# thunlp/OpenMatch

Measured on NVIDIA H100. Metric: queries/sec top-1000 over 8.8M x 768 corpus, higher is better.
Workload: dtype f16

## Files before the change

### openmatch_b200/csrc/scan_gemm.cuh

```cuda
#pragma once
#include <cuda_fp16.h>

#include "scan_epilogue.cuh"

namespace om {

constexpr int kScanBlockN = 256;
constexpr int kScanStages = 3;
constexpr int kScanABytes = kBlockM * kBlockK * 2;
constexpr int kScanBBytes = kScanBlockN * kBlockK * 2;
constexpr int kScanStageBytes = kScanABytes + kScanBBytes;
constexpr int kScanConsumers = 256;
constexpr int kScanStash = 4;
constexpr int kScanStashOffset = kScanStages * kScanStageBytes;
constexpr int kScanStashBytes = 2 * 2 * kScanStash * kScanConsumers * 8;
constexpr int kScanBarOffset = kScanStashOffset + kScanStashBytes;
constexpr int kScanSmemBytes = kScanBarOffset + 2 * kScanStages * 8 + 1024;
static_assert(kScanSmemBytes <= 232448, "scan ring + stash exceed the 227 KB of shared memory an H100 block may use");

template <int H>
__device__ __forceinline__ float scan_pick(const float (&acc)[128], int i) {
  float a[32], b[16], c[8], d[4], e[2];
#pragma unroll
  for (int j = 0; j < 32; ++j) a[j] = (i & 1) ? acc[4 * j + 2 * H + 1] : acc[4 * j + 2 * H];
// ... 172 lines not shown
      const int row0 = m_blk * kBlockM + frow, row1 = row0 + 8;
      const float inf = __int_as_float(0x7f800000);
      const float t0 = row0 < nq ? thr[row0] : inf, t1 = row1 < nq ? thr[row1] : inf;

      float acc[128];
#pragma unroll
      for (int i = 0; i < 128; ++i) acc[i] = 0.f;
      ring_consume(
          full_bar, ring, 0, num_k, 31,
          [&](uint32_t stage, uint32_t accumulate) {
            const uint32_t a_addr = smem_u32(smem + stage * kScanStageBytes) + wg * (64 * 128);
            const uint32_t b_addr = smem_u32(smem + stage * kScanStageBytes + kScanABytes);
#pragma unroll
            for (int k = 0; k < kBlockK / kWgmmaK; ++k)
              wgmma_m64n256k16_f16<0, 0>(acc, wgmma_desc(a_addr + k * 32, kDescKMajorSW128),
                                         wgmma_desc(b_addr + k * 32, kDescKMajorSW128), (accumulate | k) != 0 ? 1u : 0u);
          },
          release);
      wgmma_fence_regs(acc);

      drain();
      const int col0 = n_blk * kScanBlockN;
      const int lim = n_cols - col0;
      unsigned long long* sb = stash + buf * (2 * kScanStash * kScanConsumers) + et;
      const int k0 = scan_filter_row<0>(acc, t0, row0, lim, q4, col0, sb, cand, count, overflow, C, row_base);
      const int k1 = scan_filter_row<1>(acc, t1, row1, lim, q4, col0, sb + kScanStash * kScanConsumers, cand, count,
                                        overflow, C, row_base);
      if (__any_sync(0xffffffffu, (k0 | k1) != 0)) {
        int x0 = k0, x1 = k1;
        int y0 = __shfl_up_sync(0xffffffffu, x0, 1, 4), y1 = __shfl_up_sync(0xffffffffu, x1, 1, 4);
        if (q4 >= 1) x0 += y0, x1 += y1;
        y0 = __shfl_up_sync(0xffffffffu, x0, 2, 4), y1 = __shfl_up_sync(0xffffffffu, x1, 2, 4);
        if (q4 >= 2) x0 += y0, x1 += y1;
        const int n0 = __shfl_sync(0xffffffffu, x0, lane | 3), n1 = __shfl_sync(0xffffffffu, x1, lane | 3);
        if (q4 == 0) {
          if (n0 > 0) p_pos0 = atomicAdd(count + row0, n0);
          if (n1 > 0) p_pos1 = atomicAdd(count + row1, n1);
        }
        p_n0 = k0;
        p_n1 = k1;
        p_excl0 = x0 - k0;
        p_excl1 = x1 - k1;
        p_row = row0;
        p_buf = buf;
        buf ^= 1;
      }
    }
    drain();
  }

  __syncthreads();
  cluster_sync_all();
}

template <int CQ, int CX>
static inline cudaError_t scan_wide_max_clusters(int num_sms, int* out) {
  static int max_clusters = -1;
  if (max_clusters < 0) {
    constexpr int kSize = ScanCluster<CQ, CX>::kSize;
    cudaError_t e =
        cudaFuncSetAttribute(scan_wide_kernel<CQ, CX>, cudaFuncAttributeMaxDynamicSharedMemorySize, kScanSmemBytes);
    if (e != cudaSuccess) return e;
    cudaLaunchConfig_t cfg = {};
    cfg.gridDim = dim3(kSize * (num_sms / kSize));
    cfg.blockDim = dim3(kGemmProducerThreads + kScanConsumers);
    cfg.dynamicSmemBytes = kScanSmemBytes;
    cudaLaunchAttribute attr[1];
    attr[0].id = cudaLaunchAttributeClusterDimension;
    attr[0].val.clusterDim = {static_cast<unsigned>(kSize), 1, 1};
    cfg.attrs = attr;
    cfg.numAttrs = 1;
    int n = 0;
    e = cudaOccupancyMaxActiveClusters(&n, scan_wide_kernel<CQ, CX>, &cfg);
    if (e != cudaSuccess) return e;
    max_clusters = n < num_sms / kSize ? n : num_sms / kSize;
  }
  *out = max_clusters;
  return cudaSuccess;
}

template <int CQ, int CX>
static inline cudaError_t launch_scan_wide(const __half* Q, int64_t ldq, const __half* X, int64_t ldx, int nq, int n_cols,
                                           int K, const float* thr, unsigned long long* cand, int* count, int* overflow,
                                           int C, uint32_t row_base, int num_sms, cudaStream_t stream) {
  using Cl = ScanCluster<CQ, CX>;
  CUtensorMap tmQ, tmX;
  if (make_tmap_bf16_2d(&tmQ, Q, (uint64_t)K, (uint64_t)nq, (uint64_t)ldq * 2, kBlockK, Cl::kQRows) != 0)
    return cudaErrorInvalidValue;
  if (make_tmap_bf16_2d(&tmX, X, (uint64_t)K, (uint64_t)n_cols, (uint64_t)ldx * 2, kBlockK, Cl::kXRows) != 0)
    return cudaErrorInvalidValue;
  int max_clusters = 0;
  cudaError_t e = scan_wide_max_clusters<CQ, CX>(num_sms, &max_clusters);
  if (e != cudaSuccess) return e;
  if (max_clusters < 1) return cudaErrorNotSupported;
  cudaLaunchConfig_t cfg = {};
  cfg.blockDim = dim3(kGemmProducerThreads + kScanConsumers);
  cfg.dynamicSmemBytes = kScanSmemBytes;
  cfg.stream = stream;
  cudaLaunchAttribute attr[1];
  attr[0].id = cudaLaunchAttributeClusterDimension;
  attr[0].val.clusterDim = {static_cast<unsigned>(Cl::kSize), 1, 1};
  cfg.attrs = attr;
  cfg.numAttrs = 1;
  const int qgroups = (nq + CQ * kBlockM - 1) / (CQ * kBlockM);
  const int64_t num_tiles = static_cast<int64_t>(qgroups) * ((n_cols + CX * kScanBlockN - 1) / (CX * kScanBlockN));
  const int clusters = num_tiles < max_clusters ? static_cast<int>(num_tiles) : max_clusters;
  cfg.gridDim = dim3(Cl::kSize * clusters);
  return cudaLaunchKernelEx(&cfg, scan_wide_kernel<CQ, CX>, tmQ, tmX, K, thr, cand, count, overflow, nq, n_cols, C,
                            row_base);
}

static inline cudaError_t launch_scan_cluster(int cq, int cx, const __half* Q, int64_t ldq, const __half* X, int64_t ldx,
                                              int nq, int n_cols, int K, const float* thr, unsigned long long* cand,
                                              int* count, int* overflow, int C, uint32_t row_base, int num_sms,
                                              cudaStream_t stream) {
  if (nq <= 0 || n_cols <= 0 || K <= 0) return cudaSuccess;
  if (cq == 2 && cx == 1)
    return launch_scan_wide<2, 1>(Q, ldq, X, ldx, nq, n_cols, K, thr, cand, count, overflow, C, row_base, num_sms, stream);
  if (cq == 4 && cx == 1)
    return launch_scan_wide<4, 1>(Q, ldq, X, ldx, nq, n_cols, K, thr, cand, count, overflow, C, row_base, num_sms, stream);
  if (cq == 2 && cx == 2)
    return launch_scan_wide<2, 2>(Q, ldq, X, ldx, nq, n_cols, K, thr, cand, count, overflow, C, row_base, num_sms, stream);
  if (cq == 4 && cx == 2)
    return launch_scan_wide<4, 2>(Q, ldq, X, ldx, nq, n_cols, K, thr, cand, count, overflow, C, row_base, num_sms, stream);
  return cudaErrorInvalidValue;
}

static inline cudaError_t scan_cluster_capacity(int cq, int cx, int num_sms, int* out) {
  *out = -1;
  if (cq == 2 && cx == 1) return scan_wide_max_clusters<2, 1>(num_sms, out);
  if (cq == 4 && cx == 1) return scan_wide_max_clusters<4, 1>(num_sms, out);
  if (cq == 2 && cx == 2) return scan_wide_max_clusters<2, 2>(num_sms, out);
  if (cq == 4 && cx == 2) return scan_wide_max_clusters<4, 2>(num_sms, out);
  return cudaSuccess;
}

}
```

### openmatch_b200/csrc/search.cu

```cuda
#include <cuda_fp16.h>
#include <float.h>
#include <math.h>
#include <stdlib.h>
#include <string.h>

#include <algorithm>
#include <new>
#include <vector>

#include "common.h"
#include "gemm.cuh"
#include "nccl_dyn.h"
#include "scan_epilogue.cuh"
#include "scan_gemm.cuh"

namespace om {

__device__ __forceinline__ void bitonic_sort_desc(unsigned long long* s, int P, int tid, int nthreads) {
  for (int k = 2; k <= P; k <<= 1) {
    for (int j = k >> 1; j > 0; j >>= 1) {
      for (int t = tid; t < (P >> 1); t += nthreads) {
        const int i = ((t & ~(j - 1)) << 1) | (t & (j - 1));
        const int p = i | j;
        const unsigned long long a = s[i], b = s[p];
// ... 460 lines not shown
                                   float* __restrict__ dst) {
  for (int64_t i = blockIdx.x * static_cast<int64_t>(blockDim.x) + threadIdx.x; i < static_cast<int64_t>(n) * d;
       i += static_cast<int64_t>(gridDim.x) * blockDim.x) {
    const int r = static_cast<int>(i / d);
    dst[i] = src[static_cast<size_t>(list[r]) * d + (i - static_cast<int64_t>(r) * d)];
  }
}
__global__ void scatter_results_kernel(const float* __restrict__ Dsub, const int64_t* __restrict__ Isub,
                                       const int* __restrict__ list, int n, int k, float* __restrict__ D,
                                       int64_t* __restrict__ I) {
  for (int64_t i = blockIdx.x * static_cast<int64_t>(blockDim.x) + threadIdx.x; i < static_cast<int64_t>(n) * k;
       i += static_cast<int64_t>(gridDim.x) * blockDim.x) {
    const int r = static_cast<int>(i / k);
    const size_t o = static_cast<size_t>(list[r]) * k + (i - static_cast<int64_t>(r) * k);
    D[o] = Dsub[i];
    I[o] = Isub[i];
  }
}
__global__ void compose_list_kernel(const int* __restrict__ outer, const int* __restrict__ inner, int n, int* out) {
  const int i = blockIdx.x * blockDim.x + threadIdx.x;
  if (i < n) out[i] = outer[inner[i]];
}

}

using namespace om;

struct om_comm {
  void* nccl = nullptr;
  int rank = 0, world = 1;
};

namespace {

constexpr int kQueryChunk = 16384;
constexpr int kMaxCandidates = 4096;

struct DevBuf {
  void* p = nullptr;
  size_t bytes = 0;
  int reserve(size_t need) {
    if (need <= bytes) return 0;
    if (p) cudaFree(p);
    p = nullptr;
    bytes = 0;
    OM_CUDA(dev_malloc(&p, need));
    bytes = need;
    return 0;
  }
  void release() {
    if (p) cudaFree(p);
    p = nullptr;
    bytes = 0;
  }
};

struct Level {
  int nq = 0, k = 0, kp = 0, kp_target = 0, C = 0, growth = 2, mode = 0, world = 1, kc = 0, nqc_max = 0;
  const float* qf = nullptr;
  __half* qh = nullptr;
  float *hn = nullptr, *en = nullptr;
  unsigned long long* cand = nullptr;
  int* count = nullptr;
  float* thr = nullptr;
  int* status = nullptr;
  uint8_t *send = nullptr, *recv = nullptr;
};

}

struct om_index {
  int d = 0, dpad = 0;
  int storage = OM_F32;
  int64_t n = 0, cap = 0;
  float* xf = nullptr;
  __half* xh = nullptr;
  float* gstats = nullptr;
  bool gstats_stale = false;
  int64_t st_nonfinite = 0;
  int64_t rescore_slack = -1;
  int force_safe = 0;
  int pair_scan = 1;
  int scan_cq = 0, scan_cx = 0;
  int growth = 0;
  int certify = 1;
  int exact_only = 0;
  int stage_scores = 0;
  int64_t st_rounds = 0, st_retries = 0, st_capacity = 0, st_launches = 0;
  int64_t st_flagged = 0, st_flagged_wide = 0, st_exact = 0;
  int64_t st_scan_cluster = 0, st_scan_clusters = 0;
  int profile = 0;
  double st_scan_us = 0, st_select_us = 0, st_final_us = 0, st_other_us = 0;
  std::vector<cudaEvent_t> ev;
  std::vector<int> ev_kind;
  size_t ev_used = 0;
  DevBuf ws, ows, sws;
  int* h_status = nullptr;
};

static int index_grow(om_index* ix, int64_t need) {
  if (need <= ix->cap) return 0;
  int64_t ncap = std::max<int64_t>(need, ix->cap + ix->cap / 2);
  ncap = round_up(std::max<int64_t>(ncap, 1024), 256);
  float* nxf = nullptr;
  __half* nxh = nullptr;
  const bool master = ix->storage == OM_F32;
  OM_CUDA(cudaDeviceSynchronize());
  if (master) OM_CUDA(dev_malloc(&nxf, static_cast<size_t>(ncap) * ix->d * sizeof(float)));
  cudaError_t e = dev_malloc(&nxh, static_cast<size_t>(ncap) * ix->dpad * sizeof(__half));
  if (e != cudaSuccess) {
    cudaFree(nxf);
    cudaGetLastError();
    return fail(OM_ENOMEM, "index: cannot allocate the fp16 rows for %lld rows", (long long)ncap);
  }
  if (ix->n > 0) {
    if (master)
      OM_CUDA(cudaMemcpy(nxf, ix->xf, static_cast<size_t>(ix->n) * ix->d * sizeof(float), cudaMemcpyDeviceToDevice));
    OM_CUDA(cudaMemcpy(nxh, ix->xh, static_cast<size_t>(ix->n) * ix->dpad * sizeof(__half), cudaMemcpyDeviceToDevice));
  }
  OM_CUDA(cudaDeviceSynchronize());
  cudaFree(ix->xf);
  cudaFree(ix->xh);
  ix->xf = nxf;
  ix->xh = nxh;
  ix->cap = ncap;
  return 0;
}

static inline int grid_for(int64_t n, int threads) {
  int64_t g = (n + threads - 1) / threads;
  return static_cast<int>(std::min<int64_t>(std::max<int64_t>(g, 1), 132 * 16));
}

static int settle_reset(om_index* ix, cudaStream_t st) {
  if (!ix->gstats_stale) return 0;
  OM_CUDA(cudaMemsetAsync(ix->gstats, 0, 3 * sizeof(float), st));
  ix->gstats_stale = false;
  return 0;
}

extern "C" {

int om_index_create(int d, om_index** out) { return om_index_create_typed(d, OM_F32, out); }

int om_index_create_typed(int d, om_dtype storage, om_index** out) {
  if (!out || d <= 0) return fail(OM_EINVAL, "om_index_create: d must be positive");
  if (storage != OM_F32 && storage != OM_F16)
    return fail(OM_EINVAL, "om_index_create_typed: storage must be OM_F32 or OM_F16 (the scan operand is fp16)");
  OM_TRY(device_sm_count());
  om_index* ix = new (std::nothrow) om_index();
  if (!ix) return fail(OM_ENOMEM, "om_index_create: out of host memory");
  ix->d = d;
  ix->dpad = static_cast<int>(round_up(d, 8));
  ix->storage = storage;
  if (cudaMalloc(&ix->gstats, 4 * sizeof(float)) != cudaSuccess || cudaMemset(ix->gstats, 0, 4 * sizeof(float)) != cudaSuccess ||
      cudaHostAlloc(&ix->h_status, 8 * sizeof(int), cudaHostAllocDefault) != cudaSuccess) {
    cudaGetLastError();
    cudaFree(ix->gstats);
    delete ix;
    return fail(OM_ENOMEM, "om_index_create: cannot allocate index state");
  }
  *out = ix;
  return 0;
}

void om_index_destroy(om_index* ix) {
  if (!ix) return;
  cudaFree(ix->xf);
  cudaFree(ix->xh);
  cudaFree(ix->gstats);
  if (ix->h_status) cudaFreeHost(ix->h_status);
  ix->ws.release();
  ix->ows.release();
  ix->sws.release();
  for (cudaEvent_t e : ix->ev) cudaEventDestroy(e);
  delete ix;
}

int64_t om_index_ntotal(const om_index* ix) { return ix ? ix->n : 0; }
int om_index_dim(const om_index* ix) { return ix ? ix->d : 0; }
int om_index_storage(const om_index* ix) { return ix ? ix->storage : fail(OM_EINVAL, "om_index_storage: null index"); }

int om_index_reset(om_index* ix) {
  if (!ix) return fail(OM_EINVAL, "om_index_reset: null index");
  ix->n = 0;
  ix->gstats_stale = true;
  ix->st_nonfinite = 0;
  return 0;
}

int om_index_reserve_rows(om_index* ix, int64_t n, void** dev_rows, int64_t* row_pitch_elems) {
  if (!ix || n < 0 || !dev_rows || !row_pitch_elems) return fail(OM_EINVAL, "om_index_reserve_rows: bad arguments");
  if (ix->n + n > 0xfffffff0ll) return fail(OM_EINVAL, "index shard limited to 2^32-16 rows; shard the corpus");
  OM_TRY(index_grow(ix, ix->n + n));
  if (ix->storage == OM_F16) {
    *dev_rows = ix->xh + static_cast<size_t>(ix->n) * ix->dpad;
    *row_pitch_elems = ix->dpad;
  } else {
    *dev_rows = ix->xf + static_cast<size_t>(ix->n) * ix->d;
    *row_pitch_elems = ix->d;
  }
  return 0;
}

int om_index_reserve(om_index* ix, int64_t n, float** dev_rows) {
  if (!ix || n < 0 || !dev_rows) return fail(OM_EINVAL, "om_index_reserve: bad arguments");
  if (ix->storage != OM_F32) return fail(OM_ESTATE, "om_index_reserve: the index stores fp16 rows; use om_index_reserve_rows");
  void* rows = nullptr;
  int64_t pitch = 0;
  OM_TRY(om_index_reserve_rows(ix, n, &rows, &pitch));
  *dev_rows = static_cast<float*>(rows);
  return 0;
}

int om_index_commit(om_index* ix, int64_t n, void* stream) {
  if (!ix || n < 0 || ix->n + n > ix->cap) return fail(OM_EINVAL, "om_index_commit: more rows than reserved");
  if (n == 0) return 0;
  cudaStream_t st = static_cast<cudaStream_t>(stream);
  OM_TRY(settle_reset(ix, st));
  if (ix->storage == OM_F16)
    commit_f16_rows_kernel<<<grid_for(n, 8), 256, 0, st>>>(ix->xh + static_cast<size_t>(ix->n) * ix->dpad, n, ix->d,
                                                           ix->dpad, ix->gstats, reinterpret_cast<int*>(ix->gstats) + 2);
  else
    rows_to_f16_kernel<<<grid_for(n, 8), 256, 0, st>>>(ix->xf + static_cast<size_t>(ix->n) * ix->d,
                                                       ix->xh + static_cast<size_t>(ix->n) * ix->dpad, n, ix->d, ix->dpad,
                                                       nullptr, nullptr, ix->gstats);
  OM_CUDA(cudaGetLastError());
  ix->n += n;
  return 0;
}

static int add_f16(om_index* ix, const void* x, om_memkind kind, om_dtype dtype, int64_t n, cudaStream_t st) {
  void* rows = nullptr;
  int64_t pitch = 0;
  OM_TRY(om_index_reserve_rows(ix, n, &rows, &pitch));
  __half* dst = static_cast<__half*>(rows);
  const size_t elems = static_cast<size_t>(n) * ix->d;
  const size_t esize = dtype == OM_F32 ? 4 : 2;
  const void* src = x;
  void* tmp = nullptr;
  if (kind == OM_HOST) {
    OM_CUDA(cudaMalloc(&tmp, elems * esize));
    OM_CUDA(cudaMemcpyAsync(tmp, x, elems * esize, cudaMemcpyHostToDevice, st));
    src = tmp;
  }
  int* bad = reinterpret_cast<int*>(ix->gstats) + 3;
  cudaError_t e = cudaMemsetAsync(bad, 0, sizeof(int), st);
  const int grid = grid_for(static_cast<int64_t>(elems), 256);
  if (e == cudaSuccess) {
    if (dtype == OM_F32)
      to_f16_rows_kernel<<<grid, 256, 0, st>>>(static_cast<const float*>(src), n, ix->d, dst, ix->dpad, bad);
    else if (dtype == OM_BF16)
      to_f16_rows_kernel<<<grid, 256, 0, st>>>(static_cast<const __nv_bfloat16*>(src), n, ix->d, dst, ix->dpad, bad);
    else
      to_f16_rows_kernel<<<grid, 256, 0, st>>>(static_cast<const __half*>(src), n, ix->d, dst, ix->dpad, bad);
    e = cudaGetLastError();
  }
  if (e == cudaSuccess) e = cudaMemcpyAsync(ix->h_status + 4, bad, sizeof(int), cudaMemcpyDeviceToHost, st);
  if (e == cudaSuccess) e = cudaStreamSynchronize(st);
  if (tmp) cudaFree(tmp);
  OM_CUDA(e);
  if (ix->h_status[4] > 0)
    return fail(OM_EINVAL, "om_index_add: %d elements are NaN or round to +-inf in fp16 (|x| >= 65520); fp16 storage cannot "
                "hold them and no row was added", ix->h_status[4]);
  return om_index_commit(ix, n, st);
}

int om_index_add(om_index* ix, const void* x, om_memkind kind, om_dtype dtype, int64_t n, void* stream) {
  if (!ix || (!x && n > 0) || n < 0) return fail(OM_EINVAL, "om_index_add: bad arguments");
  if (n == 0) return 0;
  cudaStream_t st = static_cast<cudaStream_t>(stream);
  if (ix->storage == OM_F16) {
    if (dtype != OM_F32 && dtype != OM_BF16 && dtype != OM_F16)
      return fail(OM_EINVAL, "om_index_add: unsupported dtype %d", (int)dtype);
    return add_f16(ix, x, kind, dtype, n, st);
  }
  float* dst = nullptr;
  OM_TRY(om_index_reserve(ix, n, &dst));
  const size_t elems = static_cast<size_t>(n) * ix->d;
  if (dtype == OM_F32) {
    OM_CUDA(cudaMemcpyAsync(dst, x, elems * 4, kind == OM_HOST ? cudaMemcpyHostToDevice : cudaMemcpyDeviceToDevice,
                            st));
  } else if (dtype == OM_BF16 || dtype == OM_F16) {
    const void* src = x;
    void* tmp = nullptr;
    if (kind == OM_HOST) {
      OM_CUDA(cudaMalloc(&tmp, elems * 2));
      OM_CUDA(cudaMemcpyAsync(tmp, x, elems * 2, cudaMemcpyHostToDevice, st));
      src = tmp;
    }
    if (dtype == OM_BF16)
      to_f32<<<grid_for(elems, 256), 256, 0, st>>>(static_cast<const __nv_bfloat16*>(src), dst, (int64_t)elems);
    else
      to_f32<<<grid_for(elems, 256), 256, 0, st>>>(static_cast<const __half*>(src), dst, (int64_t)elems);
    OM_CUDA(cudaGetLastError());
    if (tmp) {
      OM_CUDA(cudaStreamSynchronize(st));
      cudaFree(tmp);
    }
  } else {
    return fail(OM_EINVAL, "om_index_add: unsupported dtype %d", (int)dtype);
  }
  OM_TRY(om_index_commit(ix, n, stream));
  if (kind == OM_HOST) OM_CUDA(cudaStreamSynchronize(st));
  return 0;
}

int om_index_set_param(om_index* ix, const char* name, int64_t value) {
  if (!ix || !name) return fail(OM_EINVAL, "om_index_set_param: bad arguments");
  if (!strcmp(name, "rescore_slack")) {
    ix->rescore_slack = value;
  } else if (!strcmp(name, "force_safe_rounds")) {
    ix->force_safe = value != 0;
  } else if (!strcmp(name, "round_growth")) {
    if (value != 0 && (value < 2 || value > 8)) return fail(OM_EINVAL, "round_growth must be 0 (auto) or in [2, 8]");
    ix->growth = static_cast<int>(value);
  } else if (!strcmp(name, "pair_scan")) {
    ix->pair_scan = value != 0;
  } else if (!strcmp(name, "scan_cluster_q")) {
    if (value != 0 && value != 2 && value != 4) return fail(OM_EINVAL, "scan_cluster_q must be 0 (auto), 2 or 4");
    ix->scan_cq = static_cast<int>(value);
  } else if (!strcmp(name, "scan_cluster_x")) {
    if (value != 0 && value != 1 && value != 2) return fail(OM_EINVAL, "scan_cluster_x must be 0 (auto), 1 or 2");
    ix->scan_cx = static_cast<int>(value);
  } else if (!strcmp(name, "profile")) {
    ix->profile = static_cast<int>(value);
  } else if (!strcmp(name, "certify")) {
    ix->certify = value != 0;
  } else if (!strcmp(name, "exact_only")) {
    ix->exact_only = value != 0;
  } else if (!strcmp(name, "debug_stage_scores")) {
    ix->stage_scores = value != 0;
  } else {
    return fail(OM_EINVAL, "om_index_set_param: unknown parameter '%s'", name);
  }
  return 0;
}

int64_t om_index_get_stat(const om_index* ix, const char* name) {
  if (!ix || !name) return -1;
  if (!strcmp(name, "rounds")) return ix->st_rounds;
  if (!strcmp(name, "overflow_retries")) return ix->st_retries;
  if (!strcmp(name, "candidates")) return ix->st_capacity;
  if (!strcmp(name, "launches")) return ix->st_launches;
  if (!strcmp(name, "uncertified")) return ix->st_flagged;
  if (!strcmp(name, "uncertified_wide")) return ix->st_flagged_wide;
  if (!strcmp(name, "exact_queries")) return ix->st_exact;
  if (!strcmp(name, "nonfinite_rows")) return ix->st_nonfinite;
  if (!strcmp(name, "scan_cluster")) return ix->st_scan_cluster;
  if (!strcmp(name, "scan_max_clusters")) return ix->st_scan_clusters;
  if (!strcmp(name, "scan_ns")) return static_cast<int64_t>(ix->st_scan_us * 1e3);
  if (!strcmp(name, "select_ns")) return static_cast<int64_t>(ix->st_select_us * 1e3);
  if (!strcmp(name, "finalize_ns")) return static_cast<int64_t>(ix->st_final_us * 1e3);
  if (!strcmp(name, "other_ns")) return static_cast<int64_t>(ix->st_other_us * 1e3);
  return -1;
}

}

namespace {

struct Timed {
  om_index* ix;
  cudaStream_t st;
  bool on;
  Timed(om_index* ix_, cudaStream_t st_, int kind) : ix(ix_), st(st_), on(ix_->profile != 0) {
    static const char* nvtx_names[4] = {"om.search.scan", "om.search.select", "om.search.rescore", "om.search.exchange_certify"};
    nvtxRangePushA(nvtx_names[kind & 3]);
    if (!on) return;
    if (ix->ev_used + 2 > ix->ev.size()) {
      cudaEvent_t a, b;
      if (cudaEventCreate(&a) != cudaSuccess || cudaEventCreate(&b) != cudaSuccess) {
        on = false;
        return;
      }
      ix->ev.push_back(a);
      ix->ev.push_back(b);
      ix->ev_kind.push_back(0);
    }
    ix->ev_kind[ix->ev_used / 2] = kind;
    cudaEventRecord(ix->ev[ix->ev_used], st);
  }
  ~Timed() {
    nvtxRangePop();
    if (!on) return;
    cudaEventRecord(ix->ev[ix->ev_used + 1], st);
    ix->ev_used += 2;
  }
};

void collect_profile(om_index* ix) {
  static const char* names[4] = {"scan", "select", "finalize", "exchange+certify"};
  for (size_t i = 0; i + 1 < ix->ev_used; i += 2) {
    float ms = 0.f;
    if (cudaEventElapsedTime(&ms, ix->ev[i], ix->ev[i + 1]) != cudaSuccess) continue;
    const int kind = ix->ev_kind[i / 2];
    (kind == 0 ? ix->st_scan_us : kind == 1 ? ix->st_select_us : kind == 2 ? ix->st_final_us : ix->st_other_us) += ms * 1e3;
    if (ix->profile >= 2) fprintf(stderr, "[om profile] launch %zu %s %.3f ms\n", i / 2, names[kind & 3], ms);
  }
  ix->ev_used = 0;
}

int once_attrs() {
  static bool done = false;
  if (done) return 0;
  OM_CUDA(cudaFuncSetAttribute(select_kernel, cudaFuncAttributeMaxDynamicSharedMemorySize, 16384 * 8));
  OM_CUDA(cudaFuncSetAttribute(finalize_kernel<float>, cudaFuncAttributeMaxDynamicSharedMemorySize, kMaxCandidates * 8 + 65536));
  OM_CUDA(cudaFuncSetAttribute(finalize_kernel<__half>, cudaFuncAttributeMaxDynamicSharedMemorySize, kMaxCandidates * 8 + 65536));
  OM_CUDA(cudaFuncSetAttribute(merge_kernel, cudaFuncAttributeMaxDynamicSharedMemorySize, 8192 * 16));
  OM_CUDA(cudaFuncSetAttribute(exact_scan_kernel<8, 2, float>, cudaFuncAttributeMaxDynamicSharedMemorySize, 96 * 1024));
  OM_CUDA(cudaFuncSetAttribute(exact_scan_kernel<8, 2, __half>, cudaFuncAttributeMaxDynamicSharedMemorySize, 96 * 1024));
  done = true;
  return 0;
}

struct ExchangeBlock {
  size_t off_i, off_floor, off_stats, bytes;
};
inline ExchangeBlock exchange_block(size_t nqc, size_t kc) {
  ExchangeBlock b;
  b.off_i = round_up(nqc * kc * 4, 256);
  b.off_floor = b.off_i + round_up(nqc * kc * 8, 256);
  b.off_stats = b.off_floor + round_up(nqc * 4, 256);
  b.bytes = b.off_stats + 256;
  return b;
}
inline size_t exchange_block_bytes(size_t nqc, size_t kc) { return exchange_block(nqc, kc).bytes; }

int level_prepare(om_index* ix, Level& L, const float* qf, int nq, int k, int kp_target, int mode, int world,
                  cudaStream_t st) {
  const int d = ix->d, dpad = ix->dpad;
  if (d > 16384) return fail(OM_EINVAL, "om_index_search: d > 16384 unsupported");
  if (k > kMaxCandidates) return fail(OM_EINVAL, "om_index_search: k = %d exceeds %d", k, kMaxCandidates);
  OM_TRY(once_attrs());
  L.qf = qf;
  L.nq = nq;
  L.k = k;
  L.mode = mode;
  L.world = world;
  L.kp_target = std::min(std::max(kp_target, k), kMaxCandidates);
  if (world > 1 && mode == 0 && L.kp_target < kMaxCandidates) {
    const double m = static_cast<double>(L.kp_target) / world;
    L.kp_target = static_cast<int>(std::min<int64_t>(L.kp_target, round_up(static_cast<int64_t>(m + 6.0 * sqrt(m) + 32.0), 32)));
  }
  L.kp = static_cast<int>(std::min<int64_t>(L.kp_target, std::max<int64_t>(ix->n, 1)));
  for (L.growth = ix->growth > 0 ? ix->growth : (nq <= 256 ? 8 : 2);; --L.growth) {
    L.C = 1024;
    while (L.C < (5 * L.growth * L.kp) / 4 + 512) L.C <<= 1;
    if (L.C <= 16384 || L.growth == 2) break;
  }
  if (L.C > 16384) return fail(OM_EINVAL, "om_index_search: candidate list of %d entries exceeds 16384; lower k", L.C);
  L.kc = std::min(k, L.kp_target);
  L.nqc_max = std::min(nq, kQueryChunk);
  ix->st_capacity = L.C;
  size_t off = 0;
  auto carve = [&](size_t bytes) {
    size_t o = off;
    off += round_up(bytes, 256);
    return o;
  };
  const size_t nqc = L.nqc_max;
  const size_t o_qh = carve(static_cast<size_t>(nq) * dpad * 2), o_hn = carve(static_cast<size_t>(nq) * 4),
               o_en = carve(static_cast<size_t>(nq) * 4), o_cand = carve(nqc * L.C * 8), o_count = carve(nqc * 4),
               o_thr = carve(nqc * 4), o_status = carve(256);
  size_t o_send = 0, o_recv = 0;
  if (world > 1) {
    const size_t blk = exchange_block_bytes(nqc, L.kc);
    o_send = carve(blk);
    o_recv = carve(blk * world);
  }
  OM_TRY(ix->ws.reserve(off));
  uint8_t* base = static_cast<uint8_t*>(ix->ws.p);
  L.qh = reinterpret_cast<__half*>(base + o_qh);
  L.hn = reinterpret_cast<float*>(base + o_hn);
  L.en = reinterpret_cast<float*>(base + o_en);
  L.cand = reinterpret_cast<unsigned long long*>(base + o_cand);
  L.count = reinterpret_cast<int*>(base + o_count);
  L.thr = reinterpret_cast<float*>(base + o_thr);
  L.status = reinterpret_cast<int*>(base + o_status);
  L.send = world > 1 ? base + o_send : nullptr;
  L.recv = world > 1 ? base + o_recv : nullptr;
  if (mode == 0) {
    rows_to_f16_kernel<<<grid_for(nq, 8), 256, 0, st>>>(qf, L.qh, nq, d, dpad, L.hn, L.en, nullptr);
    OM_CUDA(cudaGetLastError());
    ix->st_launches += 1;
  }
  return 0;
}

int sweep_chunk(om_index* ix, const Level& L, int q0, int nqc, bool safe, int sms, cudaStream_t st) {
  const int64_t growth = L.growth;
  const int64_t N = ix->n;
  const int C = L.C, kp = L.kp;
  if (N == 0) {
    fill_i32<<<(nqc + 255) / 256, 256, 0, st>>>(L.count, 0, nqc);
    fill_i32<<<(nqc + 255) / 256, 256, 0, st>>>(reinterpret_cast<int*>(L.thr), static_cast<int>(0xff800000), nqc);
    OM_CUDA(cudaGetLastError());
    return 0;
  }
  const __half* qh = L.qh + static_cast<size_t>(q0) * ix->dpad;
  const float* qf = L.qf + static_cast<size_t>(q0) * ix->d;
  int* overflow = L.status;
  int64_t pos = 0;
  const size_t sel_smem = static_cast<size_t>(C) * 8;
  bool first = true;
  while (pos < N) {
    int64_t step;
    if (first)
      step = std::min<int64_t>(N, C);
    else if (safe)
      step = std::min<int64_t>(N - pos, std::max<int64_t>(256, ((C - kp) / 256) * 256));
    else
      step = std::min<int64_t>(N - pos, (growth - 1) * pos);
    {
      Timed t(ix, st, 0);
      if (L.mode == 0) {
        const __half* xrows = ix->xh + static_cast<size_t>(pos) * ix->dpad;
        cudaError_t e;
        const int ncols = static_cast<int>(step);
        const bool pair = ix->pair_scan != 0 && nqc > kBlockM;
        if (first) {
          EpiScan<true> epi{L.thr, L.cand, L.count, overflow, nqc, ncols, C, static_cast<uint32_t>(pos)};
          e = launch_gemm<128, 3, true, EpiScan<true>, true>(qh, ix->dpad, xrows, ix->dpad, nqc, ncols, ix->d, epi, sms, st, true);
        } else if (pair) {
          const int cq = ix->scan_cq ? ix->scan_cq : 2, cx = ix->scan_cx ? ix->scan_cx : 1;
          int clusters = 0;
          e = launch_scan_cluster(cq, cx, qh, ix->dpad, xrows, ix->dpad, nqc, ncols, ix->d, L.thr, L.cand, L.count,
                                  overflow, C, static_cast<uint32_t>(pos), sms, st);
          if (e == cudaSuccess) e = scan_cluster_capacity(cq, cx, sms, &clusters);
          ix->st_scan_cluster = 10 * cq + cx;
          ix->st_scan_clusters = clusters;
        } else {
          EpiScan<false> epi{L.thr, L.cand, L.count, overflow, nqc, ncols, C, static_cast<uint32_t>(pos)};
          e = launch_gemm<128, 3, true, EpiScan<false>, true>(qh, ix->dpad, xrows, ix->dpad, nqc, ncols, ix->d, epi, sms, st, true);
        }
        if (e != cudaSuccess) return fail(OM_ECUDA, "scan kernel launch failed: %s", cudaGetErrorString(e));
      } else {
        const int nqt = std::max(1, std::min(8, (96 * 1024) / (ix->d * 4)));
        dim3 grid(static_cast<unsigned>(std::min<int64_t>((step + 15) / 16, static_cast<int64_t>(sms) * 4)),
                  static_cast<unsigned>((nqc + nqt - 1) / nqt));
        const size_t smem = static_cast<size_t>(nqt) * ix->d * 4;
        if (ix->storage == OM_F16)
          exact_scan_kernel<8, 2><<<grid, 256, smem, st>>>(ix->xh + static_cast<size_t>(pos) * ix->dpad, step,
                                                           static_cast<uint32_t>(pos), qf, nqc, ix->d, nqt, L.thr, L.cand,
                                                           L.count, overflow, C, first ? 1 : 0);
        else
          exact_scan_kernel<8, 2><<<grid, 256, smem, st>>>(ix->xf + static_cast<size_t>(pos) * ix->d, step,
                                                           static_cast<uint32_t>(pos), qf, nqc, ix->d, nqt, L.thr, L.cand,
                                                           L.count, overflow, C, first ? 1 : 0);
        OM_CUDA(cudaGetLastError());
      }
    }
    {
      Timed t(ix, st, 1);
      select_kernel<<<nqc, 256, sel_smem, st>>>(L.cand, L.count, L.thr, C, kp, first ? static_cast<int>(step) : -1);
    }
    OM_CUDA(cudaGetLastError());
    ix->st_launches += 2;
    pos += step;
    first = false;
    ix->st_rounds++;
  }
  return 0;
}

int finalize_chunk(om_index* ix, const Level& L, int q0, int nqc, float* D, int64_t* I, int k_out, int64_t id_offset,
                   cudaStream_t st) {
  int P2 = 2;
  while (P2 < L.kp) P2 <<= 1;
  const size_t fin_smem = static_cast<size_t>(P2) * 8 + static_cast<size_t>(ix->d) * 4;
  {
    Timed t(ix, st, 2);
    const float* qf = L.qf + static_cast<size_t>(q0) * ix->d;
    if (ix->storage == OM_F16)
      finalize_kernel<<<nqc, 256, fin_smem, st>>>(L.cand, L.count, L.C, qf, ix->xh, ix->d, D, I, id_offset, k_out,
                                                  ix->stage_scores);
    else
      finalize_kernel<<<nqc, 256, fin_smem, st>>>(L.cand, L.count, L.C, qf, ix->xf, ix->d, D, I, id_offset, k_out,
                                                  ix->stage_scores);
  }
  OM_CUDA(cudaGetLastError());
  ix->st_launches += 1;
  return 0;
}

#define OM_NCCL(expr)                                                                                   \
  do {                                                                                                  \
    int r__ = (expr);                                                                                   \
    if (r__ != 0) return fail(OM_ECUDA, "%s failed: %s", #expr, nccl_api().GetErrorString(r__));        \
  } while (0)

int merge_parts(const float* Dp, const int64_t* Ip, int64_t stride_d, int64_t stride_i, int nparts, int nq, int k_in,
                int k_out, float* D, int64_t* I, cudaStream_t st) {
  OM_TRY(once_attrs());
  if (k_in > 8192) return fail(OM_EINVAL, "om_topk_merge_n: k_in = %d exceeds 8192", k_in);
  if (static_cast<int64_t>(nparts) * k_in <= 8192) {
    int P = 2;
    while (P < nparts * k_in) P <<= 1;
    const size_t smem = static_cast<size_t>(P) * 8 + static_cast<size_t>(nparts) * k_in * 8;
    merge_kernel<<<nq, 256, smem, st>>>(Dp, Ip, stride_d, stride_i, nparts, nq, k_in, k_out, D, I);
    OM_CUDA(cudaGetLastError());
    return 0;
  }
  if (k_in > 4096 || k_out > 4096)
    return fail(OM_EINVAL, "om_topk_merge_n: %d parts x %d entries exceed one merge of 8192 and need k_in, k_out <= 4096 "
                "(got k_in = %d, k_out = %d)", nparts, k_in, k_in, k_out);
  const int g = std::max(2, 8192 / k_in);
  const int ngroups = (nparts + g - 1) / g;
  const int k_mid = static_cast<int>(std::min<int64_t>(k_out, static_cast<int64_t>(g) * k_in));
  float* Dm = nullptr;
  int64_t* Im = nullptr;
  const size_t per = static_cast<size_t>(nq) * k_mid;
  OM_CUDA(cudaMallocAsync(&Dm, per * ngroups * 4, st));
  OM_CUDA(cudaMallocAsync(&Im, per * ngroups * 8, st));
// ... 27 lines not shown
  }
  ix->st_launches += 2;
  return 0;
}

int run_level(om_index* ix, om_comm* comm, Level& L, float* dD, int64_t* dI, int64_t id_offset, int* flags,
              int* flag_list, int* nflag_out, cudaStream_t st) {
  const int sms = device_sm_count();
  if (sms < 0) return sms;
  NvtxRange nvtx(L.mode == 1 ? "om.search.level_exact" : (L.kp_target >= kMaxCandidates ? "om.search.level_wide" : "om.search.level0"));
  const bool sharded = comm && comm->world > 1;
  bool safe = ix->force_safe != 0;
  const bool certify = ix->certify && L.mode == 0 && flags != nullptr && !ix->stage_scores;
  for (int attempt = 0; attempt < 4; ++attempt) {
    OM_CUDA(cudaMemsetAsync(L.status, 0, 32, st));
    for (int q0 = 0; q0 < L.nq; q0 += kQueryChunk) {
      const int nqc = std::min(kQueryChunk, L.nq - q0);
      OM_TRY(sweep_chunk(ix, L, q0, nqc, safe, sms, st));
      if (sharded)
        OM_TRY(exchange_chunk(ix, comm, L, q0, nqc, dD, dI, id_offset, st));
      else
        OM_TRY(finalize_chunk(ix, L, q0, nqc, dD + static_cast<size_t>(q0) * L.k, dI + static_cast<size_t>(q0) * L.k, L.k,
                              id_offset, st));
      if (certify) {
        Timed t(ix, st, 3);
        const ExchangeBlock b = exchange_block(nqc, L.kc);
        const float* floors = sharded ? reinterpret_cast<const float*>(L.recv + b.off_floor) : L.thr;
        const float* gst = sharded ? reinterpret_cast<const float*>(L.recv + b.off_stats) : ix->gstats;
        certify_kernel<<<(nqc + 7) / 8, 256, 0, st>>>(dD + static_cast<size_t>(q0) * L.k, dI + static_cast<size_t>(q0) * L.k,
                                                      L.k, floors, static_cast<int64_t>(b.bytes / 4), sharded ? comm->world : 1,
                                                      gst, static_cast<int64_t>(b.bytes / 4), L.hn + q0, L.en + q0, ix->d, nqc,
                                                      q0, flags, L.status + 2);
        OM_CUDA(cudaGetLastError());
        ix->st_launches += 1;
      }
    }
    if (sharded)
      OM_NCCL(nccl_api().AllReduce(L.status, L.status, 1, kNcclInt32, kNcclMax, comm->nccl, st));
    OM_CUDA(cudaMemcpyAsync(ix->h_status, L.status, 4 * sizeof(int), cudaMemcpyDeviceToHost, st));
    OM_CUDA(cudaStreamSynchronize(st));
    const unsigned int fault = read_clear_dev_fault();
    if (fault) return fail(OM_EFAULT, "scan kernel pipeline fault 0x%08x", fault);
    if (ix->h_status[0]) {
      if (safe) return fail(OM_EFAULT, "candidate list overflow in the overflow-proof schedule (bug)");
      safe = true;
      ix->st_retries++;
      continue;
    }
    *nflag_out = certify ? ix->h_status[2] : 0;
    if (*nflag_out > 0) {
      compact_flags_kernel<<<1, 1024, 0, st>>>(flags, L.nq, flag_list);
      OM_CUDA(cudaGetLastError());
      ix->st_launches += 1;
    }
    return 0;
  }
  return fail(OM_EFAULT, "search level did not converge (bug)");
}

int check_finite_rows(om_index* ix, om_comm* comm, cudaStream_t st) {
  if (ix->storage != OM_F16) return 0;
  int* cnt = reinterpret_cast<int*>(ix->gstats) + 2;
  const bool sharded = comm && comm->world > 1;
  if (sharded) OM_NCCL(nccl_api().AllReduce(cnt, cnt + 1, 1, kNcclInt32, kNcclSum, comm->nccl, st));
  OM_CUDA(cudaMemcpyAsync(ix->h_status + 4, cnt, 2 * sizeof(int), cudaMemcpyDeviceToHost, st));
  OM_CUDA(cudaStreamSynchronize(st));
  ix->st_nonfinite = ix->h_status[4];
  const int total = sharded ? ix->h_status[5] : ix->h_status[4];
  if (total > 0)
    return fail(OM_EINVAL, "search: %d committed fp16 rows hold inf or NaN (%d on this shard); fp16 storage cannot answer "
                "exactly over them: reset the index", total, ix->h_status[4]);
  return 0;
}

int search_impl(om_index* ix, om_comm* comm, const void* q, om_memkind q_kind, int nq, int k, float* D, int64_t* I,
                om_memkind out_kind, int64_t id_offset, cudaStream_t st) {
  NvtxRange nvtx("om.search");
  const int d = ix->d;
  const int world = comm ? comm->world : 1;
  ix->st_rounds = ix->st_retries = ix->st_launches = 0;
  ix->st_flagged = ix->st_flagged_wide = ix->st_exact = 0;
  ix->st_scan_cluster = ix->st_scan_clusters = 0;
  ix->st_scan_us = ix->st_select_us = ix->st_final_us = ix->st_other_us = 0;
  ix->ev_used = 0;
  OM_TRY(check_finite_rows(ix, comm, st));
  size_t off = 0;
  auto carve = [&](size_t bytes) {
    size_t o = off;
    off += round_up(bytes, 256);
    return o;
  };
  const size_t o_q = carve(q_kind == OM_HOST ? static_cast<size_t>(nq) * d * 4 : 0);
  const size_t o_D = carve(out_kind == OM_HOST ? static_cast<size_t>(nq) * k * 4 : 0);
  const size_t o_I = carve(out_kind == OM_HOST ? static_cast<size_t>(nq) * k * 8 : 0);
  const size_t o_flags = carve(static_cast<size_t>(nq) * 4);
  const size_t o_flag = carve(static_cast<size_t>(nq) * 4);
  const size_t o_sub = carve(static_cast<size_t>(nq) * 4);
  const size_t o_flag2 = carve(static_cast<size_t>(nq) * 4);
  OM_TRY(ix->ows.reserve(off));
  uint8_t* ob = static_cast<uint8_t*>(ix->ows.p);
  const float* qf = static_cast<const float*>(q);
  if (q_kind == OM_HOST) {
    OM_CUDA(cudaMemcpyAsync(ob + o_q, q, static_cast<size_t>(nq) * d * 4, cudaMemcpyHostToDevice, st));
    qf = reinterpret_cast<const float*>(ob + o_q);
  }
  float* dD = out_kind == OM_HOST ? reinterpret_cast<float*>(ob + o_D) : D;
  int64_t* dI = out_kind == OM_HOST ? reinterpret_cast<int64_t*>(ob + o_I) : I;
  int* flags = reinterpret_cast<int*>(ob + o_flags);
  int* flag_list = reinterpret_cast<int*>(ob + o_flag);
  int* sub_flags = reinterpret_cast<int*>(ob + o_sub);
  int* flag_list2 = reinterpret_cast<int*>(ob + o_flag2);

  const int64_t slack = ix->rescore_slack >= 0 ? ix->rescore_slack : std::max<int64_t>(128, k / 5);
  const int kp0 = static_cast<int>(std::min<int64_t>(static_cast<int64_t>(k) + slack, kMaxCandidates));
  int nf = 0;
  if (!ix->exact_only) {
    Level L;
    OM_TRY(level_prepare(ix, L, qf, nq, k, kp0, 0, world, st));
    OM_TRY(run_level(ix, comm, L, dD, dI, id_offset, flags, flag_list, &nf, st));
    ix->st_flagged = nf;
  }
  auto run_sub = [&](const int* list, int n_sub, int kp_target, int mode, int* nf_out) -> int {
    Level Ls;
    if (!list) {
      OM_TRY(level_prepare(ix, Ls, qf, n_sub, k, kp_target, mode, world, st));
      return run_level(ix, comm, Ls, dD, dI, id_offset, flags, sub_flags, nf_out, st);
    }
    size_t so = 0;
    auto scarve = [&](size_t bytes) {
      size_t o = so;
      so += round_up(bytes, 256);
      return o;
    };
    const size_t s_q = scarve(static_cast<size_t>(n_sub) * d * 4), s_D = scarve(static_cast<size_t>(n_sub) * k * 4),
                 s_I = scarve(static_cast<size_t>(n_sub) * k * 8);
    OM_TRY(ix->sws.reserve(so));
    uint8_t* sb = static_cast<uint8_t*>(ix->sws.p);
    float* qsub = reinterpret_cast<float*>(sb + s_q);
    float* Ds = reinterpret_cast<float*>(sb + s_D);
    int64_t* Is = reinterpret_cast<int64_t*>(sb + s_I);
    gather_rows_kernel<<<grid_for(static_cast<int64_t>(n_sub) * d, 256), 256, 0, st>>>(qf, list, n_sub, d, qsub);
    OM_CUDA(cudaGetLastError());
    OM_TRY(level_prepare(ix, Ls, qsub, n_sub, k, kp_target, mode, world, st));
    OM_TRY(run_level(ix, comm, Ls, Ds, Is, id_offset, flags, sub_flags, nf_out, st));
    scatter_results_kernel<<<grid_for(static_cast<int64_t>(n_sub) * k, 256), 256, 0, st>>>(Ds, Is, list, n_sub, k, dD, dI);
    OM_CUDA(cudaGetLastError());
    ix->st_launches += 2;
    return 0;
  };
  if (ix->exact_only) {
    int dummy = 0;
    ix->st_exact = nq;
    OM_TRY(run_sub(nullptr, nq, k, 1, &dummy));
  } else if (nf > 0) {
    const int* list = flag_list;
    if (kp0 < kMaxCandidates && (world > 1 || ix->n > kp0)) {
      int nf1 = 0;
      OM_TRY(run_sub(list, nf, kMaxCandidates, 0, &nf1));
      if (nf1 > 0) {
        compose_list_kernel<<<(nf1 + 255) / 256, 256, 0, st>>>(list, sub_flags, nf1, flag_list2);
        OM_CUDA(cudaGetLastError());
        list = flag_list2;
      }
      nf = nf1;
    }
    ix->st_flagged_wide = nf;
// ... 83 lines not shown
```

Baseline: 38140.

## Split scan columns between wide 4x2 clusters and concurrent 2x1 clusters on a side stream

The scan kernel now runs by default as a mixed launch. A 4x2 cluster kernel on the main stream covers the first share of corpus rows. A 2x1 cluster kernel on a side stream covers the rest, capped to the SMs left after the wide clusters are placed. The split is proportional to the SMs each part gets and can be overridden per mille. The aim is to use the larger-cluster tile's better operand reuse while filling the SMs that 8-CTA clusters cannot pack. The cost is fork/join events, assumptions about two kernels running concurrently, and possible load imbalance between the two parts.

```diff
diff --git a/openmatch_b200/csrc/scan_gemm.cuh b/openmatch_b200/csrc/scan_gemm.cuh
--- a/openmatch_b200/csrc/scan_gemm.cuh
+++ b/openmatch_b200/csrc/scan_gemm.cuh
@@ -278,7 +278,7 @@
 template <int CQ, int CX>
 static inline cudaError_t launch_scan_wide(const __half* Q, int64_t ldq, const __half* X, int64_t ldx, int nq, int n_cols,
                                            int K, const float* thr, unsigned long long* cand, int* count, int* overflow,
-                                           int C, uint32_t row_base, int num_sms, cudaStream_t stream) {
+                                           int C, uint32_t row_base, int num_sms, int cluster_limit, cudaStream_t stream) {
   using Cl = ScanCluster<CQ, CX>;
   CUtensorMap tmQ, tmX;
   if (make_tmap_bf16_2d(&tmQ, Q, (uint64_t)K, (uint64_t)nq, (uint64_t)ldq * 2, kBlockK, Cl::kQRows) != 0)
@@ -289,6 +289,7 @@
   cudaError_t e = scan_wide_max_clusters<CQ, CX>(num_sms, &max_clusters);
   if (e != cudaSuccess) return e;
   if (max_clusters < 1) return cudaErrorNotSupported;
+  if (cluster_limit > 0 && cluster_limit < max_clusters) max_clusters = cluster_limit;
   cudaLaunchConfig_t cfg = {};
   cfg.blockDim = dim3(kGemmProducerThreads + kScanConsumers);
   cfg.dynamicSmemBytes = kScanSmemBytes;
@@ -309,16 +310,16 @@
 static inline cudaError_t launch_scan_cluster(int cq, int cx, const __half* Q, int64_t ldq, const __half* X, int64_t ldx,
                                               int nq, int n_cols, int K, const float* thr, unsigned long long* cand,
                                               int* count, int* overflow, int C, uint32_t row_base, int num_sms,
-                                              cudaStream_t stream) {
+                                              int cluster_limit, cudaStream_t stream) {
   if (nq <= 0 || n_cols <= 0 || K <= 0) return cudaSuccess;
   if (cq == 2 && cx == 1)
-    return launch_scan_wide<2, 1>(Q, ldq, X, ldx, nq, n_cols, K, thr, cand, count, overflow, C, row_base, num_sms, stream);
+    return launch_scan_wide<2, 1>(Q, ldq, X, ldx, nq, n_cols, K, thr, cand, count, overflow, C, row_base, num_sms, cluster_limit, stream);
   if (cq == 4 && cx == 1)
-    return launch_scan_wide<4, 1>(Q, ldq, X, ldx, nq, n_cols, K, thr, cand, count, overflow, C, row_base, num_sms, stream);
+    return launch_scan_wide<4, 1>(Q, ldq, X, ldx, nq, n_cols, K, thr, cand, count, overflow, C, row_base, num_sms, cluster_limit, stream);
   if (cq == 2 && cx == 2)
-    return launch_scan_wide<2, 2>(Q, ldq, X, ldx, nq, n_cols, K, thr, cand, count, overflow, C, row_base, num_sms, stream);
+    return launch_scan_wide<2, 2>(Q, ldq, X, ldx, nq, n_cols, K, thr, cand, count, overflow, C, row_base, num_sms, cluster_limit, stream);
   if (cq == 4 && cx == 2)
-    return launch_scan_wide<4, 2>(Q, ldq, X, ldx, nq, n_cols, K, thr, cand, count, overflow, C, row_base, num_sms, stream);
+    return launch_scan_wide<4, 2>(Q, ldq, X, ldx, nq, n_cols, K, thr, cand, count, overflow, C, row_base, num_sms, cluster_limit, stream);
   return cudaErrorInvalidValue;
 }
 
diff --git a/openmatch_b200/csrc/search.cu b/openmatch_b200/csrc/search.cu
--- a/openmatch_b200/csrc/search.cu
+++ b/openmatch_b200/csrc/search.cu
@@ -566,6 +566,10 @@
   int force_safe = 0;
   int pair_scan = 1;
   int scan_cq = 0, scan_cx = 0;
+  int scan_mixed = 1;
+  int scan_mixed_split = -1;
+  cudaStream_t side = nullptr;
+  cudaEvent_t ev_fork = nullptr, ev_join = nullptr;
   int growth = 0;
   int certify = 1;
   int exact_only = 0;
@@ -573,8 +577,10 @@
   int64_t st_rounds = 0, st_retries = 0, st_capacity = 0, st_launches = 0;
   int64_t st_flagged = 0, st_flagged_wide = 0, st_exact = 0;
   int64_t st_scan_cluster = 0, st_scan_clusters = 0;
+  int64_t st_scan_mixed = 0, st_scan_mixed_clusters = 0;
   int profile = 0;
   double st_scan_us = 0, st_select_us = 0, st_final_us = 0, st_other_us = 0;
+  double st_scan_wide_us = 0, st_scan_pair_us = 0;
   std::vector<cudaEvent_t> ev;
   std::vector<int> ev_kind;
   size_t ev_used = 0;
@@ -658,6 +664,9 @@
   ix->ows.release();
   ix->sws.release();
   for (cudaEvent_t e : ix->ev) cudaEventDestroy(e);
+  if (ix->side) cudaStreamDestroy(ix->side);
+  if (ix->ev_fork) cudaEventDestroy(ix->ev_fork);
+  if (ix->ev_join) cudaEventDestroy(ix->ev_join);
   delete ix;
 }
 
@@ -807,6 +816,13 @@
   } else if (!strcmp(name, "scan_cluster_x")) {
     if (value != 0 && value != 1 && value != 2) return fail(OM_EINVAL, "scan_cluster_x must be 0 (auto), 1 or 2");
     ix->scan_cx = static_cast<int>(value);
+  } else if (!strcmp(name, "scan_mixed")) {
+    if (value != 0 && value != 1 && value != 41 && value != 42)
+      return fail(OM_EINVAL, "scan_mixed must be 0 (off), 1 (on) or the wide shape 41 (4 x 1) or 42 (4 x 2)");
+    ix->scan_mixed = static_cast<int>(value);
+  } else if (!strcmp(name, "scan_mixed_split")) {
+    if (value < -1 || value > 1000) return fail(OM_EINVAL, "scan_mixed_split must be -1 (default) or in [0, 1000] per mille");
+    ix->scan_mixed_split = static_cast<int>(value);
   } else if (!strcmp(name, "profile")) {
     ix->profile = static_cast<int>(value);
   } else if (!strcmp(name, "certify")) {
@@ -833,6 +849,10 @@
   if (!strcmp(name, "nonfinite_rows")) return ix->st_nonfinite;
   if (!strcmp(name, "scan_cluster")) return ix->st_scan_cluster;
   if (!strcmp(name, "scan_max_clusters")) return ix->st_scan_clusters;
+  if (!strcmp(name, "scan_mixed")) return ix->st_scan_mixed;
+  if (!strcmp(name, "scan_mixed_clusters")) return ix->st_scan_mixed_clusters;
+  if (!strcmp(name, "scan_wide_ns")) return static_cast<int64_t>(ix->st_scan_wide_us * 1e3);
+  if (!strcmp(name, "scan_pair_ns")) return static_cast<int64_t>(ix->st_scan_pair_us * 1e3);
   if (!strcmp(name, "scan_ns")) return static_cast<int64_t>(ix->st_scan_us * 1e3);
   if (!strcmp(name, "select_ns")) return static_cast<int64_t>(ix->st_select_us * 1e3);
   if (!strcmp(name, "finalize_ns")) return static_cast<int64_t>(ix->st_final_us * 1e3);
@@ -848,9 +868,11 @@
   om_index* ix;
   cudaStream_t st;
   bool on;
+  size_t slot = 0;
   Timed(om_index* ix_, cudaStream_t st_, int kind) : ix(ix_), st(st_), on(ix_->profile != 0) {
-    static const char* nvtx_names[4] = {"om.search.scan", "om.search.select", "om.search.rescore", "om.search.exchange_certify"};
-    nvtxRangePushA(nvtx_names[kind & 3]);
+    static const char* nvtx_names[6] = {"om.search.scan", "om.search.select", "om.search.rescore", "om.search.exchange_certify",
+                                        "om.search.scan_wide", "om.search.scan_pairs"};
+    nvtxRangePushA(nvtx_names[kind]);
     if (!on) return;
     if (ix->ev_used + 2 > ix->ev.size()) {
       cudaEvent_t a, b;
@@ -862,25 +884,28 @@
       ix->ev.push_back(b);
       ix->ev_kind.push_back(0);
     }
-    ix->ev_kind[ix->ev_used / 2] = kind;
-    cudaEventRecord(ix->ev[ix->ev_used], st);
+    slot = ix->ev_used;
+    ix->ev_used += 2;
+    ix->ev_kind[slot / 2] = kind;
+    cudaEventRecord(ix->ev[slot], st);
   }
   ~Timed() {
     nvtxRangePop();
     if (!on) return;
-    cudaEventRecord(ix->ev[ix->ev_used + 1], st);
-    ix->ev_used += 2;
+    cudaEventRecord(ix->ev[slot + 1], st);
   }
 };
 
 void collect_profile(om_index* ix) {
-  static const char* names[4] = {"scan", "select", "finalize", "exchange+certify"};
+  static const char* names[6] = {"scan", "select", "finalize", "exchange+certify", "scan wide part", "scan 2x1 part"};
   for (size_t i = 0; i + 1 < ix->ev_used; i += 2) {
     float ms = 0.f;
     if (cudaEventElapsedTime(&ms, ix->ev[i], ix->ev[i + 1]) != cudaSuccess) continue;
     const int kind = ix->ev_kind[i / 2];
-    (kind == 0 ? ix->st_scan_us : kind == 1 ? ix->st_select_us : kind == 2 ? ix->st_final_us : ix->st_other_us) += ms * 1e3;
-    if (ix->profile >= 2) fprintf(stderr, "[om profile] launch %zu %s %.3f ms\n", i / 2, names[kind & 3], ms);
+    double* acc[6] = {&ix->st_scan_us, &ix->st_select_us, &ix->st_final_us, &ix->st_other_us, &ix->st_scan_wide_us,
+                      &ix->st_scan_pair_us};
+    *acc[kind] += ms * 1e3;
+    if (ix->profile >= 2) fprintf(stderr, "[om profile] launch %zu %s %.3f ms\n", i / 2, names[kind], ms);
   }
   ix->ev_used = 0;
 }
@@ -970,6 +995,61 @@
     ix->st_launches += 1;
   }
   return 0;
+}
+
+constexpr int kMixedWide = 42;
+
+cudaError_t scan_wide_round(om_index* ix, const Level& L, const __half* qh, const __half* xrows, int nqc, int ncols,
+                            uint32_t row_base, int sms, cudaStream_t st) {
+  const int cq = ix->scan_cq ? ix->scan_cq : 2, cx = ix->scan_cx ? ix->scan_cx : 1;
+  int clusters = 0;
+  cudaError_t e = scan_cluster_capacity(cq, cx, sms, &clusters);
+  if (e != cudaSuccess) return e;
+  ix->st_scan_cluster = 10 * cq + cx;
+  ix->st_scan_clusters = clusters;
+  ix->st_scan_mixed = ix->st_scan_mixed_clusters = 0;
+  const int wide = ix->scan_mixed == 1 ? kMixedWide : ix->scan_mixed, wq = wide / 10, wx = wide % 10;
+  int wn = 0;
+  if (ix->scan_mixed && !ix->scan_cq && !ix->scan_cx) {
+    e = scan_cluster_capacity(wq, wx, sms, &wn);
+    if (e != cudaSuccess) return e;
+  }
+  const int tile_rows = kScanBlockN * wx, wsms = wq * wx * wn;
+  const int64_t wide_tiles =
+      static_cast<int64_t>((nqc + wq * kBlockM - 1) / (wq * kBlockM)) * ((ncols + tile_rows - 1) / tile_rows);
+  if (wn < 1 || wide_tiles < wn)
+    return launch_scan_cluster(cq, cx, qh, ix->dpad, xrows, ix->dpad, nqc, ncols, ix->d, L.thr, L.cand, L.count, L.status, L.C,
+                               row_base, sms, 0, st);
+  const int pairs = (sms - wsms) / 2;
+  const double share = pairs < 1 ? 1.0
+                       : ix->scan_mixed_split >= 0 ? ix->scan_mixed_split / 1000.0
+                       : static_cast<double>(wsms) / (wsms + 2.0 * pairs);
+  const int split =
+      share >= 1.0 ? ncols : static_cast<int>(std::min<int64_t>(ncols, llround(ncols * share / tile_rows) * tile_rows));
+  if (!ix->side) {
+    if ((e = cudaStreamCreateWithFlags(&ix->side, cudaStreamNonBlocking)) != cudaSuccess ||
+        (e = cudaEventCreateWithFlags(&ix->ev_fork, cudaEventDisableTiming)) != cudaSuccess ||
+        (e = cudaEventCreateWithFlags(&ix->ev_join, cudaEventDisableTiming)) != cudaSuccess)
+      return e;
+  }
+  ix->st_scan_mixed = wide;
+  ix->st_scan_mixed_clusters = wn;
+  if ((e = cudaEventRecord(ix->ev_fork, st)) != cudaSuccess || (e = cudaStreamWaitEvent(ix->side, ix->ev_fork, 0)) != cudaSuccess)
+    return e;
+  {
+    Timed t(ix, st, 4);
+    e = launch_scan_cluster(wq, wx, qh, ix->dpad, xrows, ix->dpad, nqc, split, ix->d, L.thr, L.cand, L.count, L.status, L.C,
+                            row_base, sms, 0, st);
+  }
+  if (e == cudaSuccess) {
+    Timed t(ix, ix->side, 5);
+    e = launch_scan_cluster(2, 1, qh, ix->dpad, xrows + static_cast<size_t>(split) * ix->dpad, ix->dpad, nqc, ncols - split,
+                            ix->d, L.thr, L.cand, L.count, L.status, L.C, row_base + static_cast<uint32_t>(split), sms, pairs,
+                            ix->side);
+  }
+  const cudaError_t j = cudaEventRecord(ix->ev_join, ix->side);
+  const cudaError_t w = j == cudaSuccess ? cudaStreamWaitEvent(st, ix->ev_join, 0) : j;
+  return e != cudaSuccess ? e : w;
 }
 
 int sweep_chunk(om_index* ix, const Level& L, int q0, int nqc, bool safe, int sms, cudaStream_t st) {
@@ -1007,13 +1087,7 @@
           EpiScan<true> epi{L.thr, L.cand, L.count, overflow, nqc, ncols, C, static_cast<uint32_t>(pos)};
           e = launch_gemm<128, 3, true, EpiScan<true>, true>(qh, ix->dpad, xrows, ix->dpad, nqc, ncols, ix->d, epi, sms, st, true);
         } else if (pair) {
-          const int cq = ix->scan_cq ? ix->scan_cq : 2, cx = ix->scan_cx ? ix->scan_cx : 1;
-          int clusters = 0;
-          e = launch_scan_cluster(cq, cx, qh, ix->dpad, xrows, ix->dpad, nqc, ncols, ix->d, L.thr, L.cand, L.count,
-                                  overflow, C, static_cast<uint32_t>(pos), sms, st);
-          if (e == cudaSuccess) e = scan_cluster_capacity(cq, cx, sms, &clusters);
-          ix->st_scan_cluster = 10 * cq + cx;
-          ix->st_scan_clusters = clusters;
+          e = scan_wide_round(ix, L, qh, xrows, nqc, ncols, static_cast<uint32_t>(pos), sms, st);
         } else {
           EpiScan<false> epi{L.thr, L.cand, L.count, overflow, nqc, ncols, C, static_cast<uint32_t>(pos)};
           e = launch_gemm<128, 3, true, EpiScan<false>, true>(qh, ix->dpad, xrows, ix->dpad, nqc, ncols, ix->d, epi, sms, st, true);
@@ -1207,6 +1281,8 @@
   ix->st_flagged = ix->st_flagged_wide = ix->st_exact = 0;
   ix->st_scan_cluster = ix->st_scan_clusters = 0;
   ix->st_scan_us = ix->st_select_us = ix->st_final_us = ix->st_other_us = 0;
+  ix->st_scan_wide_us = ix->st_scan_pair_us = 0;
+  ix->st_scan_mixed = ix->st_scan_mixed_clusters = 0;
   ix->ev_used = 0;
   OM_TRY(check_finite_rows(ix, comm, st));
   size_t off = 0;
```

Result: faster. 38760 (median of 6 runs) (+1.6%).
